# xavenordu/Audio-Compression

Measured on AMD Instinct MI355X. Metric: ranges matched/sec at tile_size=2048, top-K=64, higher is better.
Workload: dtype f32; 1 GPU; cfg2: 60 s 44100 Hz mono white noise, tile_size=2048, top_k=64, n_ranges=330750, n_domains=1321977; tile_size=2048, top_k=64, n_ranges=330750, n_domains=1321977, parallelism=single GPU, streams=2

## Files before the change

audio-compression_amd/csrc/fwav_topk.hip:

```cpp
#include <algorithm>
#include <cstring>
#include <type_traits>
#include "fwav_common.h"
#include "../../include/fwav.h"

#if !defined(FWAV_DEBUG_API) && (defined(FWAV_TOPK_ABL) || defined(FWAV_TOPK_APPOFF) || defined(FWAV_TOPK_CAP) || \
    defined(FWAV_TOPK_CB) || defined(FWAV_TOPK_CENT) || defined(FWAV_TOPK_CENTWIDE) || defined(FWAV_TOPK_CENT_HL) || \
    defined(FWAV_TOPK_CENT_MINQ) || defined(FWAV_TOPK_CG) || defined(FWAV_TOPK_CHAINS) || \
    defined(FWAV_TOPK_CPDBL) || defined(FWAV_TOPK_CPMIN) || defined(FWAV_TOPK_CSHARE) || defined(FWAV_TOPK_BANDB) || defined(FWAV_TOPK_CVACC) || \
    defined(FWAV_TOPK_CW) || defined(FWAV_TOPK_CWPE) || defined(FWAV_TOPK_DELTA) || defined(FWAV_TOPK_EXGROW) || \
    defined(FWAV_TOPK_EXWPE) || defined(FWAV_TOPK_FIRST) || defined(FWAV_TOPK_G) || defined(FWAV_TOPK_GROW) || \
    defined(FWAV_TOPK_HLDELTA) || defined(FWAV_TOPK_HLPRE) || defined(FWAV_TOPK_INTERLEAVE) || \
    defined(FWAV_TOPK_MAXP) || defined(FWAV_TOPK_PMAJOR) || defined(FWAV_TOPK_PRIO) || defined(FWAV_TOPK_QS) || \
    defined(FWAV_TOPK_RB) || defined(FWAV_TOPK_SEEDHALF) || defined(FWAV_TOPK_SMALLSORT) || defined(FWAV_TOPK_W) || \
    defined(FWAV_TOPK_WARM) || defined(FWAV_TOPK_WIDE_MIN) || defined(FWAV_TOPK_WIN) || defined(FWAV_TOPK_WPE) || \
    defined(FWAV_FLOOR_PILOTS) || defined(FWAV_FLOOR_RANK) || defined(FWAV_TOPK_YOUNG) || defined(FWAV_TOPK_TAIL))
#error "experiment switches build the debug library only (-DFWAV_DEBUG_API)"
#endif

namespace fwav {

typedef float floatx16 __attribute__((ext_vector_type(16)));

constexpr int kTopkWaves = 4;
constexpr int kTopkQ = 32 * kTopkWaves;
constexpr int kChunk = 256;
constexpr int kTopkThreads = 64 * kTopkWaves;

__device__ __forceinline__ uint64_t make_key(float s, int32_t idx) {
  return ((uint64_t)f2key(s) << 32) | (uint64_t)(~(uint32_t)idx);
}
__device__ __forceinline__ int32_t key_idx(uint64_t k) { return (int32_t)(~(uint32_t)(k & 0xffffffffu)); }
__device__ __forceinline__ float key_score(uint64_t k) { return key2f((uint32_t)(k >> 32)); }

template <int E>
__device__ __forceinline__ void wave_sort_desc(uint64_t (&v)[E]) {
  const int lane = threadIdx.x & 63;
  constexpr int N = E * 64;
#pragma unroll
  for (int size = 2; size <= N; size <<= 1) {
#pragma unroll
    for (int stride = size >> 1; stride > 0; stride >>= 1) {
      if (stride >= 64) {
        const int js = stride >> 6;
#pragma unroll
        for (int j = 0; j < E; ++j) {
          if ((j & js) == 0) {
            const int jp = j | js;
            const int e = j * 64 + lane;
            const bool desc = (e & size) == 0;
            uint64_t a = v[j], b = v[jp];
            bool sw = desc ? (a < b) : (a > b);
            v[j] = sw ? b : a;
            v[jp] = sw ? a : b;
          }
        }
      } else {
#pragma unroll
        for (int j = 0; j < E; ++j) {
          const int e = j * 64 + lane;
          uint64_t o = __shfl_xor(v[j], stride);
          const bool lower = (lane & stride) == 0;
          const bool desc = (e & size) == 0;
          uint64_t mx = v[j] > o ? v[j] : o;
          uint64_t mn = v[j] > o ? o : v[j];
          v[j] = (lower == desc) ? mx : mn;
        }
      }
    }
  }
}

template <int E>
__device__ __forceinline__ int tie_flags(const uint64_t (&v)[E], int n, int K) {
  const int lane = threadIdx.x & 63;
  bool in = false, bd = false;
#pragma unroll
  for (int j = 0; j < E; ++j) {
    uint64_t nx = __shfl_down(v[j], 1);
    const uint64_t first_next = __shfl(v[j + 1 < E ? j + 1 : j], 0);
    if (lane == 63) nx = j + 1 < E ? first_next : 0ull;
    const int e = j * 64 + lane;
    if (e + 1 < n && e + 1 <= K && key_score(nx) == key_score(v[j])) {
      if (e + 1 < K) in = true;
      else bd = true;
    }
  }
  return (__ballot(in) != 0ull ? 1 : 0) | (__ballot(bd) != 0ull ? 2 : 0);
}

template <int E>
__device__ __forceinline__ void record_tie(int32_t* ties, int32_t qid, int flags, const uint64_t (&v)[E], int n,
                                           int K, bool group) {
  if (ties == nullptr || flags == 0) return;
  const int lane = threadIdx.x & 63;
  int pos = 0;
  if (lane == 0) pos = atomicAdd(ties, 1);
  pos = __shfl(pos, 0);
  int32_t* rec = ties + 1 + (int64_t)kTieRec * pos;
  if (lane == 0) rec[0] = 2 * qid + ((flags >> 1) & 1);
  if (!(flags & 2)) return;
  int total = -1;
  if (group) {
    uint64_t kth = 0;
#pragma unroll
    for (int j = 0; j < E; ++j)
      if (j == ((K - 1) >> 6)) kth = __shfl(v[j], (K - 1) & 63);
    const float S = key_score(kth);
    total = 0;
#pragma unroll
    for (int j = 0; j < E; ++j) {
      const int e = j * 64 + lane;
      const bool in = e >= K && e < n && key_score(v[j]) == S;
      if (in && e - K < kTieRec - 2) rec[2 + e - K] = key_idx(v[j]);
      total += __popcll(__ballot(in));
    }
    if (total > kTieRec - 2) total = -1;
  }
  if (lane == 0) rec[1] = total;
}
template <int E>
__device__ __forceinline__ void record_tie(int32_t* ties, int32_t qid, int flags, const uint64_t (&v)[E], int n,
                                           int K) {
  record_tie<E>(ties, qid, flags, v, n, K, false);
}

template <int C>
__device__ __forceinline__ int compact(uint64_t* __restrict__ keys, int* __restrict__ cnt, float* __restrict__ theta,
                                       int ql, int K) {
  constexpr int E = C / 64;
  const int lane = threadIdx.x & 63;
  const int n = cnt[ql];
  uint64_t v[E];
#pragma unroll
  for (int j = 0; j < E; ++j) {
    const int e = j * 64 + lane;
    v[j] = e < n ? keys[ql * C + e] : 0ull;
  }
  wave_sort_desc<E>(v);
  const int tf = tie_flags<E>(v, n, K);
#pragma unroll
  for (int j = 0; j < E; ++j) {
    const int e = j * 64 + lane;
    if (e < K && e < n) keys[ql * C + e] = v[j];
  }
  const int kl = (K - 1) & 63, kj = (K - 1) >> 6;
  uint64_t kth = 0;
#pragma unroll
  for (int j = 0; j < E; ++j)
    if (j == kj) kth = __shfl(v[j], kl);
  if (lane == 0) {
    cnt[ql] = n < K ? n : K;
    theta[ql] = n >= K ? key_score(kth) : -INFINITY;
  }
  return tf;
// ... 818 lines not shown
      stat_add(11, __builtin_amdgcn_s_memrealtime() - t_l0);
    }
#pragma unroll
    for (int u = 0; u < kReplayBatch; ++u) {
      if (ct[u] < 0) break;
      floatx16 acc = __builtin_amdgcn_mfma_f32_32x32x16_f16(af[u], b, floatx16{}, 0, 0, 0);
      if constexpr (HL) {
#if FWAV_TOPK_HLPRE
        if (__ballot(fold16((int)0x80000000, acc) > int_threshold(thf - kStreamMargin)) == 0ull) continue;
#endif
        acc = __builtin_amdgcn_mfma_f32_32x32x16_f16(af[u], bl, acc, 0, 0, 0);
        acc = __builtin_amdgcn_mfma_f32_32x32x16_f16(afl[u], b, acc, 0, 0, 0);
      }
      thf = append_tile<C, STATS, SM, MODE>(acc, thf, qcnt, kept, ct[u], nd, gkeys, sm, qg, K, upd, stats, sp, emb,
                                          qv, kthp, share);
    }
    if (ct[kReplayBatch - 1] < 0) break;
  }
  return thf;
}

#ifndef FWAV_TOPK_SEEDHALF
#define FWAV_TOPK_SEEDHALF 64
#endif
constexpr int kSeedHalf = FWAV_TOPK_SEEDHALF;
constexpr int kSeedTiles = (2 * kSeedHalf + 62) / 32 + 1;
template <int MODE>
__device__ __forceinline__ float seed_limit(const _Float16* __restrict__ emb16, int64_t nd, half8 b, int64_t qrow,
                                            int64_t wbase, int K) {
  const int lane = threadIdx.x & 63;
  const int col = lane & 31;
  const int h = lane >> 5;
  const half8* afp[kSeedTiles];
  uint32_t wm[kSeedTiles];
#pragma unroll
  for (int t = 0; t < kSeedTiles; ++t) {
    const int64_t dt = wbase + 32 * t;
    const bool ok = dt >= 0 && dt < nd;
    const int64_t c = ok ? dt / kChunk : 0, tt = ok ? (dt % kChunk) / 32 : 0;
    afp[t] = reinterpret_cast<const half8*>(emb16 + ((c * 2 + h) * kChunk + col) * 8 + tt * 256);
    uint32_t m = 0;
#pragma unroll
    for (int r = 0; r < 16; ++r) {
      const int64_t d = dt + 4 * h + (r & 3) + 8 * (r >> 2);
      m |= (ok && d < nd && d >= qrow - kSeedHalf && d < qrow + kSeedHalf) ? (1u << r) : 0u;
    }
    wm[t] = m;
  }
  auto count_ge = [&](float thr) {
    int c = 0;
    half8 af[kSeedTiles];
#pragma unroll
    for (int t = 0; t < kSeedTiles; ++t) af[t] = *afp[t];
#pragma unroll
    for (int t = 0; t < kSeedTiles; ++t) {
      const floatx16 acc = __builtin_amdgcn_mfma_f32_32x32x16_f16(af[t], b, floatx16{}, 0, 0, 0);
#pragma unroll
      for (int r = 0; r < 16; ++r) c += ((wm[t] >> r) & 1u) && acc[r] >= thr ? 1 : 0;
    }
    return c + __shfl_xor(c, 32);
  };
  const bool ok = count_ge(0.0f) >= K;
  uint32_t T = 0x80000000u;
  for (int bit = 30; bit >= 12; --bit) {
    const uint32_t Tc = T | (1u << bit);
    const int c = count_ge(key2f(Tc));
    T = c >= K ? Tc : T;
  }
  return ok ? (MODE == kModeHL ? key2f(T) - kF16Delta - 2.0f * kHLDelta : key2f(T) - 2.0f * kF16Delta) : -INFINITY;
}

template <int NC, int QS, int MODE = 0>
__device__ __forceinline__ void stream_group(const _Float16* __restrict__ lda0, const half8 (&b)[QS],
                                             const int (&thi)[QS], int cbase, uint32_t (*fired)[kFifo],
                                             int (&nfired)[QS], int lane, int* sink = nullptr) {
  constexpr int NT = 8 * NC;
  constexpr int kChunkHalfs = 512 * 8;
  auto chunk_of = [](int i) { return i >> 3; };
  auto rd = [&](int i) {
    return *reinterpret_cast<const half8*>(lda0 + chunk_of(i) * kChunkHalfs + (i & 7) * 256);
  };
  half8 a[NT];
  floatx16 acc[NT][QS];
#pragma unroll
  for (int i = 0; i < 3 && i < NT; ++i) a[i] = rd(i);
#pragma unroll
  for (int s = 0; s < QS; ++s) acc[0][s] = __builtin_amdgcn_mfma_f32_32x32x16_f16(a[0], b[s], floatx16{}, 0, 0, 0);
  int r[QS][kChains];
#pragma unroll
  for (int s = 0; s < QS; ++s)
#pragma unroll
    for (int c = 0; c < kChains; ++c) r[s][c] = (int)0x80000000;
#pragma unroll
  for (int i = 0; i < NT; ++i) {
    if (i + 3 < NT) a[i + 3] = rd(i + 3);
#pragma unroll
    for (int s = 0; s < QS; ++s) {
      if (i + 1 < NT) acc[i + 1][s] = __builtin_amdgcn_mfma_f32_32x32x16_f16(a[i + 1], b[s], floatx16{}, 0, 0, 0);
      constexpr int cm = kChains - 1;
      if (MODE & 2)
        r[s][i & cm] = max(max(r[s][i & cm], __float_as_int(acc[i][s][0])), __float_as_int(acc[i][s][15]));
      else
        r[s][i & cm] = fold16(r[s][i & cm], acc[i][s]);
    }
    if (MODE != 0) {
      if (i == NT - 1) {
#pragma unroll
        for (int s = 0; s < QS; ++s)
#pragma unroll
          for (int c = 0; c < kChains; ++c) *sink ^= r[s][c];
      }
      continue;
    }
    if ((i & 7) == 7) {
#pragma unroll
      for (int s = 0; s < QS; ++s) {
        const int t = thi[s];
        int rm = r[s][0];
#pragma unroll
        for (int c = 1; c < kChains; ++c) rm = max(rm, r[s][c]);
        if (__ballot(rm > t) != 0ull) {
          uint32_t mk = 0u;
#pragma unroll
          for (int c = 0; c < kChains; ++c) mk |= __ballot(r[s][c] > t) != 0ull ? (1u << c) : 0u;
          if (lane == 0) fired[s][nfired[s] & (kFifo - 1)] = ((uint32_t)(cbase + chunk_of(i)) << 8) | mk;
          ++nfired[s];
        }
#pragma unroll
        for (int c = 0; c < kChains; ++c) r[s][c] = (int)0x80000000;
      }
    }
  }
}

__device__ __forceinline__ int ctz_mask(uint32_t x) { return __builtin_ctz(x); }
__device__ __forceinline__ int ctz_mask(uint64_t x) { return __builtin_ctzll(x); }
template <int N, int I = 0, class F>
__device__ __forceinline__ void static_for(F&& f) {
  if constexpr (I < N) {
    f(std::integral_constant<int, I>{});
    static_for<N, I + 1>(f);
  }
}

constexpr int kCentBatch = FWAV_TOPK_CB;
template <int QS>
__device__ __forceinline__ uint64_t cent_set_mask(int s) {
  static_assert(QS == 2 || QS == 4 || QS == 8, "centroid sets: 2, 4 or 8 query sets per wave");
  constexpr uint64_t m = QS == 2 ? 0x5555555555555555ull : (QS == 4 ? 0x1111111111111111ull : 0x0101010101010101ull);
  return m << s;
}
template <int QS, class RowOf>
__device__ __forceinline__ void centroid_setup(const _Float16* __restrict__ emb16, RowOf qrow_of, half8& bc,
                                               float& slack) {
  typedef float floatx8 __attribute__((ext_vector_type(8)));
  const int lane = threadIdx.x & 63;
  const int h = lane >> 5;
  auto frag = [&](int64_t r) {
    return *reinterpret_cast<const half8*>(emb16 + (((r >> 8) * 2 + h) * 256 + (r & 255)) * 8);
  };
  floatx8 sum = {0.f, 0.f, 0.f, 0.f, 0.f, 0.f, 0.f, 0.f};
  int nv = 0;
#pragma unroll
  for (int k = 0; k < QS; ++k) {
    const int64_t r = qrow_of(k);
    if (r >= 0) {
      const half8 m = frag(r);
      ++nv;
#pragma unroll
      for (int i = 0; i < 8; ++i) sum[i] += (float)m[i];
    }
  }
  half8 c;
#pragma unroll
  for (int i = 0; i < 8; ++i) c[i] = (_Float16)(nv > 0 ? sum[i] / (float)nv : 0.0f);
  float rho = 0.0f;
#pragma unroll
  for (int k = 0; k < QS; ++k) {
    const int64_t r = qrow_of(k);
    if (r >= 0) {
      const half8 m = frag(r);
      float d2 = 0.0f;
#pragma unroll
      for (int i = 0; i < 8; ++i) {
        const float d = (float)m[i] - (float)c[i];
        d2 += d * d;
      }
      rho = fmaxf(rho, __builtin_sqrtf(d2));
    }
  }
  rho += __shfl_xor(rho, 32);
  bc = c;
  slack = rho * (1.0f + 0x1p-9f) + 1e-5f;
}
template <int QS>
__device__ __forceinline__ int centroid_threshold(const float (&tv)[QS], float slack) {
  const int lane = threadIdx.x & 63;
  const int col = lane & 31;
  const int sj = col % QS, base = (lane & 32) + QS * (col / QS);
  float mn = INFINITY;
#pragma unroll
  for (int k = 0; k < QS; ++k) {
    float v = INFINITY;
#pragma unroll
    for (int s = 0; s < QS; ++s) {
      const float x = __shfl(tv[s], base + k);
      v = s == sj ? x : v;
    }
    mn = fminf(mn, v);
  }
  return int_threshold(mn - slack);
}
template <int NC, int QS>
__device__ __forceinline__ void cent_level1(const _Float16* __restrict__ lda0, half8 bc, int thc,
                                            uint64_t (&pend)[QS]) {
  constexpr int NT = 8 * NC;
  static_assert(NT <= 64, "tile masks are 64-bit");
  constexpr int kChunkHalfs = 512 * 8;
  auto rd = [&](int i) {
    return *reinterpret_cast<const half8*>(lda0 + (i >> 3) * kChunkHalfs + (i & 7) * 256);
  };
#pragma unroll
  for (int s = 0; s < QS; ++s) pend[s] = 0ull;
  half8 a[NT];
  floatx16 acc[NT];
#pragma unroll
  for (int i = 0; i < 3 && i < NT; ++i) a[i] = rd(i);
  acc[0] = __builtin_amdgcn_mfma_f32_32x32x16_f16(a[0], bc, floatx16{}, 0, 0, 0);
if constexpr (FWAV_TOPK_CVACC && NT <= 32) {
  uint32_t bits = 0u;
#pragma unroll
  for (int i = 0; i < NT; ++i) {
    if (i + 3 < NT) a[i + 3] = rd(i + 3);
    if (i + 1 < NT) acc[i + 1] = __builtin_amdgcn_mfma_f32_32x32x16_f16(a[i + 1], bc, floatx16{}, 0, 0, 0);
    const uint64_t m = __ballot(fold16((int)0x80000000, acc[i]) > thc);
    uint64_t co;
    asm("v_addc_co_u32_e64 %0, %1, %2, %2, %3" : "=v"(bits), "=s"(co) : "v"(bits), "s"(m));
  }
#pragma unroll
  for (int off = QS; off < 64; off <<= 1) bits |= (uint32_t)__shfl_xor((int)bits, off);
#pragma unroll
  for (int s = 0; s < QS; ++s)
    pend[s] = (uint64_t)(__builtin_bitreverse32((uint32_t)__builtin_amdgcn_readlane((int)bits, s)) >> (32 - NT));
} else {
#pragma unroll
  for (int i = 0; i < NT; ++i) {
    if (i + 3 < NT) a[i + 3] = rd(i + 3);
    if (i + 1 < NT) acc[i + 1] = __builtin_amdgcn_mfma_f32_32x32x16_f16(a[i + 1], bc, floatx16{}, 0, 0, 0);
    const uint64_t m = __ballot(fold16((int)0x80000000, acc[i]) > thc);
#pragma unroll
    for (int s = 0; s < QS; ++s)
      if (m & cent_set_mask<QS>(s)) pend[s] |= 1ull << i;
  }
}
}

template <int C, bool STATS, int MODE, int W = k16Waves, int G = kGroup, int QS = k16Sets, bool CENT = false>
__global__ __launch_bounds__(64 * W, MODE == kModeEX ? FWAV_TOPK_EXWPE : (CENT ? FWAV_TOPK_CWPE : FWAV_TOPK_WPE)) void k_sim_topk_f16(const _Float16* __restrict__ emb16,
                                                                const float* __restrict__ emb, int64_t nd,
                                                                const int32_t* __restrict__ active,
                                                                const int32_t* __restrict__ n_active_p,
                                                                int64_t q_offset, int K, int32_t* __restrict__ cand,
                                                                uint64_t* __restrict__ gkeys_all,
                                                                int32_t* __restrict__ ovf_list,
                                                                int32_t* __restrict__ n_ovf,
                                                                uint32_t* __restrict__ share_lim,
                                                                const uint32_t* __restrict__ seeds_in,
                                                                float seed_shift, int plan_rt,
                                                                int plan_p, int dbg, unsigned long long* gstats,
                                                                SgemvSplit sp, int32_t* __restrict__ ties,
                                                                FloorCtl fl) {
  constexpr bool EX = MODE == kModeEX;
  constexpr bool HL = MODE == kModeHL;
  constexpr int NG = W * QS;
  constexpr bool ABL = STATS || FWAV_TOPK_ABL != 0;
  constexpr int NB = 2;
  struct Lds {
    u32x4 slots[NB * G][512];
    Topk16SmemT<NG, STATS, !CENT, W> sm;
  };
  __shared__ __attribute__((aligned(16))) Lds lds_all;
  u32x4(*slots)[512] = lds_all.slots;
  Topk16SmemT<NG, STATS, !CENT, W>& sm = lds_all.sm;

  const int n_active = *n_active_p;
  constexpr int QB = 32 * NG;
  const uint32_t fkey = (!EX && fl.key != nullptr) ? __builtin_amdgcn_readfirstlane(*fl.key) : 0u;
  const bool alt = fl.key != nullptr && fkey == 0u;
  const TopkPlan plan = make_plan(n_active, alt ? fl.alt_rt : plan_rt, alt ? fl.alt_p : plan_p, QB);
  int64_t block;
  int piece, npieces, qhalf;
  plan_item(plan, blockIdx.x, block, piece, npieces, qhalf);
  if (block >= plan.nb) return;
  const int Wact = qhalf < 0 ? W : W / 2;
  if ((int)(threadIdx.x >> 6) >= Wact) return;
  const int qslot0 = qhalf > 0 ? (W / 2) * QS * 32 : 0;
  uint64_t* gkeys = gkeys_all + (size_t)blockIdx.x * 32 * NG * C;
  const unsigned long long t_kernel = STATS ? __builtin_amdgcn_s_memrealtime() : 0;

  const int tid = threadIdx.x;
  const int lane = tid & 63;
  const int wave = __builtin_amdgcn_readfirstlane(tid >> 6);
  unsigned long long* stats = nullptr;
  if (STATS) {
    if (lane < kStats) sm.wstat[wave][lane] = 0;
    stats = sm.wstat[wave];
  }
  const int col = lane & 31;
  const int h = lane >> 5;
  if (!STATS) dbg = FWAV_TOPK_ABL;
  half8 b[QS], bl[QS];
  float thf[QS];
  int upd[QS];
  float qv[QS][EX ? 16 : 1];
  const int64_t n16 = (int64_t)cdiv(nd, kChunk) * kChunk * 16;
  const _Float16* emb16lo = emb16 + n16;
  uint64_t kth[QS];
  float inseed[QS];
  int32_t qpos[QS];
  uint32_t* share = (npieces > 1 && !EX) ? share_lim : nullptr;
#pragma unroll
  for (int s = 0; s < QS; ++s) {
    const int ql = (wave * QS + s) * 32 + col;
    const int64_t qi = slot_query(block, qslot0 + ql, plan.nb, QB);
    const int32_t q = qi < n_active ? active[qi] : -1;
    const int64_t qrow = (int64_t)(q < 0 ? 0 : q) + q_offset;
    b[s] = *reinterpret_cast<const half8*>(emb16 + (((qrow >> 8) * 2 + h) * 256 + (qrow & 255)) * 8);
    bl[s] = *reinterpret_cast<const half8*>(emb16lo + (((qrow >> 8) * 2 + h) * 256 + (qrow & 255)) * 8);
    upd[s] = (q >= 0 && !(dbg & 1)) ? 1 : 0;
    thf[s] = upd[s] ? -INFINITY : INFINITY;
    qpos[s] = (int32_t)(qi < n_active ? qi : 0);
    if (h == 0) {
      sm.ovf[ql] = 0;
      sm.tie[ql] = 0;
      sm.qrow[ql] = qrow;
      sm.qpos[ql] = qpos[s];
    }
    kth[s] = 0ull;
    inseed[s] = seeds_in != nullptr && q >= 0 ? key2f(seeds_in[qi]) - seed_shift : -INFINITY;
    if constexpr (EX) {
      const float* qp = emb + qrow * 16;
#pragma unroll
      for (int i = 0; i < 16; ++i) qv[s][i] = qp[i];
    }
  }

  if (!(ABL && (dbg & 8192))) {
#pragma unroll
    for (int s = 0; s < QS; ++s) {
      const int64_t wbase =
          (int64_t)((__builtin_amdgcn_readfirstlane((int)sm.qrow[(wave * QS + s) * 32]) - kSeedHalf) >> 5) << 5;
      const float seed = seed_limit<MODE>(emb16, nd, b[s], sm.qrow[(wave * QS + s) * 32 + col], wbase, K);
      if (upd[s]) thf[s] = seed;
      if (STATS && (dbg & 32768) && gstats != nullptr && h == 0 && upd[s])
        gstats[16 + slot_query(block, qslot0 + (wave * QS + s) * 32 + col, plan.nb, QB)] = __float_as_uint(seed);
    }
  }
  if (seeds_in != nullptr) {
#pragma unroll
    for (int s = 0; s < QS; ++s)
      if (upd[s]) thf[s] = fmaxf(thf[s], inseed[s]);
  }
  if (fkey != 0u) {
#pragma unroll
    for (int s = 0; s < QS; ++s)
      if (upd[s]) thf[s] = fmaxf(thf[s], key2f(fkey));
  }
  int lid[QS];
#pragma unroll
  for (int s = 0; s < QS; ++s) lid[s] = wave * QS + s;
  half8 bc{};
  float cslack = 0.0f;
  auto setup_centroids = [&]() {
    const int sj = col % QS, mcol0 = QS * (col / QS);
    int ls = lid[0];
#pragma unroll
    for (int s = 1; s < QS; ++s) ls = sj == s ? lid[s] : ls;
    centroid_setup<QS>(emb16, [&](int k) -> int64_t {
      const int64_t qi = slot_query(block, qslot0 + ls * 32 + mcol0 + k, plan.nb, QB);
      return qi < n_active ? (int64_t)active[qi] + q_offset : (int64_t)-1;
    }, bc, cslack);
  };
  if constexpr (CENT) setup_centroids();
  const int nchunks = (int)cdiv(nd, kChunk);
  if ((FWAV_TOPK_PRIO & 1) && wave >= W / 2) __builtin_amdgcn_s_setprio(1);
  int c0, c1;
  piece_chunks(plan, block, piece, npieces, nchunks, c0, c1);
  const int ngroups = (c1 - c0 + G - 1) / G;
  const u32x4* src = reinterpret_cast<const u32x4*>(emb16);
  auto issue_group = [&](int gg) {
#pragma unroll
    for (int j = 0; j < G; ++j) {
      int c_ = c0 + gg * G + j;
      c_ = c_ < c1 ? c_ : c1 - 1;
      if (ABL && (dbg & 4)) c_ = 0;
      if (ABL && (dbg & 128) && (j & 1)) continue;
      for (int k = wave; k < 8; k += Wact) {
        const unsigned lds_dst = __builtin_amdgcn_readfirstlane((unsigned)(size_t)(
            (__attribute__((address_space(3))) void*)(&slots[(gg % NB) * G + j][k * 64])));
        const u32x4* gsrc = src + (int64_t)c_ * 512 + k * 64 + lane;
        unsigned keep;
        asm volatile("s_mov_b32 %0, m0\n\ts_mov_b32 m0, %2\n\ts_nop 0\n\tglobal_load_lds_dwordx4 %1, off\n\ts_mov_b32 m0, %0"
                     : "=&s"(keep) : "v"(gsrc), "s"(lds_dst) : "memory");
      }
    }
  };
  __builtin_amdgcn_s_waitcnt(0x0F70);
  if (ngroups > 0) issue_group(0);

  int sink = 0;
  int nfired[QS];
  ReplayCursor cur[QS];
  int qcnt[QS];
  int kept[QS];
#pragma unroll
  for (int s = 0; s < QS; ++s) {
    nfired[s] = qcnt[s] = kept[s] = 0;
    cur[s] = ReplayCursor{0, 0, 0u};
  }
  uint32_t shv[QS];
  for (int g = 0; g < ngroups; ++g) {
    u32x4(*half)[512] = slots + (g % NB) * G;
    const int cg = c0 + g * G;
    const int c_end = cg + G < c1 ? cg + G : c1;
    const bool window_end =
        (c_end - c0 <= kWarmChunks) || ((g + 1) % (kWindowGroups * 4 / G) == 0) || (g + 1 == ngroups);
    if (CENT && FWAV_TOPK_CSHARE && share != nullptr) {
#pragma unroll
      for (int s = 0; s < QS; ++s)
        shv[s] = __hip_atomic_load(share + qpos[s], __ATOMIC_RELAXED, __HIP_MEMORY_SCOPE_AGENT);
    }
    const unsigned long long t_b0 = STATS ? __builtin_amdgcn_s_memrealtime() : 0;
    if (!(ABL && (dbg & 256))) {
      asm volatile("s_waitcnt vmcnt(0) lgkmcnt(0)" ::: "memory");
      if (STATS) stat_add(12, __builtin_amdgcn_s_memrealtime() - t_b0);
      if (FWAV_TOPK_PRIO & 4) __builtin_amdgcn_s_setprio(0);
      if (!(ABL && (dbg & 16384))) __builtin_amdgcn_s_barrier();
      asm volatile("" ::: "memory");
    }
    const unsigned long long t_b1 = STATS ? __builtin_amdgcn_s_memrealtime() : 0;
    if (STATS) stat_add(7, t_b1 - t_b0);
    if (CENT && FWAV_TOPK_CSHARE && share != nullptr) {
#pragma unroll
      for (int s = 0; s < QS; ++s)
        if (upd[s] && shv[s] != 0u) thf[s] = fmaxf(thf[s], key2f(shv[s]));
    }
    if (g + 1 < ngroups) issue_group(g + 1);
    if (ABL && (dbg & 2)) continue;
    int thi[QS];
#pragma unroll
    for (int s = 0; s < QS; ++s) thi[s] = int_threshold(HL ? thf[s] - kStreamMargin : thf[s]);
    const _Float16* lda0 = reinterpret_cast<const _Float16*>(half[0]) + ((h * kChunk) + col) * 8;
    if constexpr (CENT) {
      float tv[QS];
#pragma unroll
      for (int s = 0; s < QS; ++s) tv[s] = HL ? thf[s] - kStreamMargin : thf[s];
      const int thc = centroid_threshold<QS>(tv, cslack);
      uint64_t pend[QS];
      const unsigned long long t_l1 = STATS ? __builtin_amdgcn_s_memrealtime() : 0;
      if (c_end - cg == G) {
        cent_level1<G, QS>(lda0, bc, thc, pend);
      } else {
#pragma unroll
        for (int s = 0; s < QS; ++s) pend[s] = 0ull;
        for (int c = cg; c < c_end; ++c) {
          uint64_t pc[QS];
          cent_level1<1, QS>(lda0 + (c - cg) * 512 * 8, bc, thc, pc);
#pragma unroll
          for (int s = 0; s < QS; ++s) pend[s] |= pc[s] << (8 * (c - cg));
        }
      }
      if (STATS) {
        stat_add(13, __builtin_amdgcn_s_memrealtime() - t_l1);
        unsigned long long np = 0;
#pragma unroll
        for (int s = 0; s < QS; ++s) np += __popcll(pend[s]);
        stat_add(14, np);
      }
      if (FWAV_TOPK_PRIO & 4) __builtin_amdgcn_s_setprio(1);
      static_for<QS>([&](auto sc) {
        constexpr int s = decltype(sc)::value;
        using TMask = uint64_t;
        TMask pm = (TMask)pend[s];
        TMask pass = 0;
        while (pm != 0) {
          int t[kCentBatch];
          bool on[kCentBatch];
#pragma unroll
          for (int u = 0; u < kCentBatch; ++u) {
            on[u] = pm != 0;
            t[u] = on[u] ? ctz_mask(pm) : t[0];
            if (on[u]) pm &= pm - 1;
          }
          half8 af[kCentBatch];
          floatx16 acc[kCentBatch];
#pragma unroll
          for (int u = 0; u < kCentBatch; ++u)
            af[u] = *reinterpret_cast<const half8*>(lda0 + (t[u] >> 3) * (512 * 8) + (t[u] & 7) * 256);
#pragma unroll
          for (int u = 0; u < kCentBatch; ++u)
            acc[u] = __builtin_amdgcn_mfma_f32_32x32x16_f16(af[u], b[s], floatx16{}, 0, 0, 0);
#pragma unroll
          for (int u = 0; u < kCentBatch; ++u) {
            if (!on[u]) break;
            if constexpr (HL) {
              if (__ballot(fold16((int)0x80000000, acc[u]) > thi[s]) != 0ull) pass |= (TMask)1 << t[u];
            } else {
              const int64_t dt = (int64_t)(cg + (t[u] >> 3)) * kChunk + (t[u] & 7) * 32;
              thf[s] = append_tile<C, STATS, Topk16SmemT<NG, STATS, !CENT, W>, MODE>(acc[u], thf[s], qcnt[s], kept[s],
                                                                                 dt, nd, gkeys, sm, lid[s], K,
                                                                                 upd[s], stats, sp, emb, qv[s],
                                                                                 &kth[s], share);
            }
          }
        }
        if constexpr (HL) {
          while (pass != 0) {
            int t[kReplayBatch];
            bool on[kReplayBatch];
#pragma unroll
            for (int u = 0; u < kReplayBatch; ++u) {
              on[u] = pass != 0;
              t[u] = on[u] ? ctz_mask(pass) : t[0];
              if (on[u]) pass &= pass - 1;
            }
            half8 afl[kReplayBatch];
#pragma unroll
            for (int u = 0; u < kReplayBatch; ++u)
              afl[u] = tile_fragment(emb16lo, (int64_t)(cg + (t[u] >> 3)) * kChunk + (t[u] & 7) * 32, h, col);
#pragma unroll
            for (int u = 0; u < kReplayBatch; ++u) {
              if (!on[u]) break;
              const half8 af = *reinterpret_cast<const half8*>(lda0 + (t[u] >> 3) * (512 * 8) + (t[u] & 7) * 256);
              floatx16 a2 = __builtin_amdgcn_mfma_f32_32x32x16_f16(af, b[s], floatx16{}, 0, 0, 0);
              a2 = __builtin_amdgcn_mfma_f32_32x32x16_f16(af, bl[s], a2, 0, 0, 0);
              a2 = __builtin_amdgcn_mfma_f32_32x32x16_f16(afl[u], b[s], a2, 0, 0, 0);
              const int64_t dt = (int64_t)(cg + (t[u] >> 3)) * kChunk + (t[u] & 7) * 32;
              thf[s] = append_tile<C, STATS, Topk16SmemT<NG, STATS, !CENT, W>, MODE>(a2, thf[s], qcnt[s], kept[s], dt,
                                                                                 nd, gkeys, sm, lid[s], K,
                                                                                 upd[s], stats, sp, emb, qv[s],
                                                                                 &kth[s], share);
            }
          }
        }
      });
    } else if (ABL && (dbg & (512 | 1024)) && c_end - cg == G) {
      if (dbg & 1024)
        stream_group<G, QS, 2>(lda0, b, thi, cg, sm.fired + wave * QS, nfired, lane, &sink);
      else
        stream_group<G, QS, 1>(lda0, b, thi, cg, sm.fired + wave * QS, nfired, lane, &sink);
    } else if (c_end - cg == G) {
      stream_group<G, QS>(lda0, b, thi, cg, sm.fired + wave * QS, nfired, lane);
    } else {
      for (int c = cg; c < c_end; ++c)
        stream_group<1, QS>(lda0 + (c - cg) * 512 * 8, b, thi, c, sm.fired + wave * QS, nfired, lane);
    }
    const unsigned long long t_c = STATS ? __builtin_amdgcn_s_memrealtime() : 0;
    if (STATS) stat_add(9, t_c - t_b1);
    if (window_end) {
      if (share != nullptr && !(CENT && FWAV_TOPK_CSHARE)) {
#pragma unroll
        for (int s = 0; s < QS; ++s) {
          const uint32_t v = __hip_atomic_load(share + qpos[s], __ATOMIC_RELAXED, __HIP_MEMORY_SCOPE_AGENT);
          if (upd[s] && v != 0u) thf[s] = fmaxf(thf[s], key2f(v));
        }
      }
      if (!CENT && (FWAV_TOPK_PRIO & 8)) __builtin_amdgcn_s_setprio(1);
      static_for<QS>([&](auto sc) {
        constexpr int s = decltype(sc)::value;
        if constexpr (!CENT) {
          if (nfired[s] > cur[s].head || cur[s].rem != 0u)
            thf[s] = replay_window<C, STATS, Topk16SmemT<NG, STATS, !CENT, W>, MODE>(emb16, emb16lo, b[s], bl[s], thf[s],
                                             qcnt[s], kept[s], cur[s], nfired[s], nd, gkeys, sm, lid[s], K, upd[s],
                                             stats, sp, emb, qv[s], &kth[s], share);
        }
      });
      if (!CENT && (FWAV_TOPK_PRIO & 8)) __builtin_amdgcn_s_setprio(0);
      if (STATS) stat_add(4, __builtin_amdgcn_s_memrealtime() - t_c);
      __builtin_amdgcn_s_waitcnt(0x0F70);
    }
  }
  const unsigned long long t_final = STATS ? __builtin_amdgcn_s_memrealtime() : 0;
#pragma unroll
  for (int s = 0; s < QS; ++s) {
    if (h == 0)
      sm.cnt[lid[s] * 32 + col] = qcnt[s];
    else
      sm.cnt1[lid[s] * 32 + col] = qcnt[s];
  }

  auto slot_of = [&](int l) {
    int ls = lid[0];
#pragma unroll
    for (int s = 1; s < QS; ++s) ls = (l >> 5) == s ? lid[s] : ls;
    return ls * 32 + (l & 31);
  };
  if (npieces > 1) {
    asm volatile("s_waitcnt vmcnt(0)" ::: "memory");
    for (int l0 = 0; l0 < 32 * QS; l0 += kBandBatch) {
      uint64_t v[kBandBatch][C / 64];
      int nb_[kBandBatch];
      uint32_t sh[kBandBatch];
#pragma unroll
      for (int b = 0; b < kBandBatch; ++b) {
        const int qs = slot_of(l0 + b);
        const int64_t qq = slot_query(block, qslot0 + qs, plan.nb, QB);
        const bool ok = l0 + b < 32 * QS && qq < n_active;
        nb_[b] = ok ? piece_band_load<C>(gkeys + (size_t)qs * C, sm, qs, v[b]) : -1;
        sh[b] = ok ? __hip_atomic_load(share_lim + qq, __ATOMIC_RELAXED, __HIP_MEMORY_SCOPE_AGENT) : 0u;
      }
#pragma unroll
      for (int b = 0; b < kBandBatch; ++b) {
        if (nb_[b] < 0) continue;
        const int qs = slot_of(l0 + b);
        const int64_t qq = slot_query(block, qslot0 + qs, plan.nb, QB);
        if (lane == 0) FWAV_TRACE(sm.qrow[qs], 3u, (uint32_t)sm.cnt[qs], (uint32_t)sm.ovf[qs], (uint32_t)sm.cnt1[qs]);
        piece_band<C, HL>(gkeys + (size_t)qs * C, sm, qs, K, share_lim + qq, v[b], nb_[b], sh[b]);
      }
    }
  }
  for (int l = 0; l < (npieces > 1 ? 0 : 32 * QS); ++l) {
    const int qs = slot_of(l);
    const int64_t qq = slot_query(block, qslot0 + qs, plan.nb, QB);
    if (qq >= n_active) continue;
    const int32_t qid = active[qq];
    uint64_t* kq = gkeys + (size_t)qs * C;
    if (lane == 0) FWAV_TRACE(sm.qrow[qs], 3u, (uint32_t)sm.cnt[qs], (uint32_t)sm.ovf[qs], (uint32_t)sm.cnt1[qs]);
    compact16<C>(kq, sm, qs, K, emb, cand + (int64_t)qid * K, sp, ties, qid, fkey, fl);
    if (lane == 0 && sm.ovf[qs]) {
      const int pos = atomicAdd(n_ovf, 1);
      ovf_list[pos] = qid;
      reinterpret_cast<uint32_t*>(n_ovf + 1)[pos] = (uint32_t)sm.ovf[qs];
    }
  }
  if (ABL && sink == 0x7fffffff) cand[0] = sink;
  if (STATS) {
    stat_add(8, __builtin_amdgcn_s_memrealtime() - t_final);
    stat_add(6, __builtin_amdgcn_s_memrealtime() - t_kernel);
    __syncthreads();
    if (gstats != nullptr && threadIdx.x == 0) {
      unsigned long long mx = 0;
      for (int w = 0; w < Wact; ++w) mx = max(mx, sm.wstat[w][6] - sm.wstat[w][7]);
      atomicAdd(gstats + 15, mx);
    }
    if (gstats != nullptr && lane < kStats && lane != 15) atomicAdd(gstats + lane, sm.wstat[wave][lane]);
    if (gstats != nullptr && (dbg & 4096) && lane == 0) {
      atomicMin(gstats + 16 + 2 * blockIdx.x, t_kernel);
      atomicMax(gstats + 17 + 2 * blockIdx.x, __builtin_amdgcn_s_memrealtime());
    }
  }
}

template <int E>
__device__ __forceinline__ void merge_band(const uint64_t* __restrict__ sw, int mb, int K, const float* __restrict__ emb,
                                           int64_t qrow, const SgemvSplit& sp, int32_t* __restrict__ ties, int32_t qid,
                                           int32_t* __restrict__ out, uint32_t fkey, const FloorCtl& fl) {
  const int lane = threadIdx.x & 63;
  uint64_t v[E];
#pragma unroll
  for (int j = 0; j < E; ++j) {
    const int e = j * 64 + lane;
    v[j] = e < mb ? sw[e] : 0ull;
  }
  const float4* qp = reinterpret_cast<const float4*>(emb + qrow * 16);
  float qv[16];
#pragma unroll
  for (int i = 0; i < 4; ++i) {
    const float4 x = qp[i];
    qv[4 * i] = x.x; qv[4 * i + 1] = x.y; qv[4 * i + 2] = x.z; qv[4 * i + 3] = x.w;
  }
#pragma unroll
  for (int j0 = 0; j0 < E; j0 += 2) {
    float4 row[2][4];
    int32_t dd[2];
#pragma unroll
    for (int jj = 0; jj < 2; ++jj) {
      const int j = j0 + jj < E ? j0 + jj : E - 1;
      dd[jj] = (j0 + jj < E && v[j] != 0ull) ? key_idx(v[j]) : 0;
      const float4* rp = reinterpret_cast<const float4*>(emb + (int64_t)dd[jj] * 16);
#pragma unroll
      for (int i = 0; i < 4; ++i) row[jj][i] = rp[i];
    }
#pragma unroll
    for (int jj = 0; jj < 2; ++jj) {
      const int j = j0 + jj;
      if (j < E && v[j] != 0ull) {
        const float acc = sgemv16([&](int k) { return f4c(row[jj][k >> 2], k & 3); }, [&](int k) { return qv[k]; },
                                  sgemv_kind((uint32_t)dd[jj], sp));
        v[j] = make_key(acc, dd[jj]);
      }
    }
  }
  wave_sort_desc<E>(v);
  if (fkey != 0u) {
// ... 1086 lines not shown
```

Measured before the change: 25.33 million ranges/s.

## Tighten centroid pruning bound with direction decomposition and cache the threshold

Replaces the plain radius slack of the centroid lower bound with a tighter bound that splits each query's offset from the centroid into a part along the centroid and a part perpendicular to it. The aim is a higher centroid threshold, so fewer tiles pass level-1 filtering and need per-query MFMA and top-k appends. It also caches the centroid threshold and recomputes it only when some query's running threshold changed, which costs extra ballots after each append. The new bound adds per-setup arithmetic and relies on careful floating-point safety margins to stay exact.

```diff
diff --git a/audio-compression_amd/csrc/fwav_centroid_bound.h b/audio-compression_amd/csrc/fwav_centroid_bound.h
--- /dev/null
+++ b/audio-compression_amd/csrc/fwav_centroid_bound.h
@@ -0,0 +1,87 @@
+#ifndef FWAV_CENTROID_BOUND_H
+#define FWAV_CENTROID_BOUND_H
+
+#include <cmath>
+
+#if defined(__HIPCC__) || defined(__CUDACC__)
+#define FWAV_HD __host__ __device__
+#else
+#define FWAV_HD
+#endif
+
+namespace fwav {
+
+constexpr float kCentD = 1.0f + 0x1p-9f;
+constexpr float kCentEta = 1e-5f;
+
+struct CentHead {
+  float n2, rho, beta, perp2;
+};
+struct CentBound {
+  float slack, gd, k0, k2;
+};
+
+FWAV_HD inline float cent_rcp(float x) {
+#if defined(__HIP_DEVICE_COMPILE__)
+  return __builtin_amdgcn_rcpf(x);
+#else
+  return 1.0f / x;
+#endif
+}
+FWAV_HD inline float cent_sqrt(float x) {
+#if defined(__HIP_DEVICE_COMPILE__)
+  return __builtin_amdgcn_sqrtf(x);
+#else
+  return sqrtf(x);
+#endif
+}
+
+FWAV_HD inline void cent_head_begin(CentHead& t, const float (&c)[8]) {
+  float n2 = 0.0f;
+  for (int i = 0; i < 8; ++i) n2 += c[i] * c[i];
+  t = CentHead{n2, 0.0f, 0.0f, 0.0f};
+}
+FWAV_HD inline void cent_head_member(CentHead& t, const float (&c)[8], const float (&q)[8]) {
+  float e2 = 0.0f, ec = 0.0f;
+  for (int i = 0; i < 8; ++i) {
+    const float e = q[i] - c[i];
+    e2 += e * e;
+    ec += e * c[i];
+  }
+  const float en = sqrtf(e2);
+  t.rho = fmaxf(t.rho, en);
+  float b2 = 0.0f;
+  if (t.n2 > 0.0f) {
+    b2 = fminf(ec * ec / t.n2, e2);
+    t.beta = fmaxf(t.beta, sqrtf(b2) + 0x1p-20f * en);
+  }
+  t.perp2 = fmaxf(t.perp2, (e2 - b2) + 0x1p-18f * e2);
+}
+FWAV_HD inline CentBound cent_bound(const CentHead& h0, const CentHead& h1) {
+  CentBound b;
+  b.slack = (h0.rho + h1.rho) * kCentD + kCentEta;
+  const float N2 = (h0.n2 + h1.n2) * (1.0f - 0x1p-20f);
+  const float s2 = (h0.perp2 + h1.perp2) * (1.0f + 0x1p-20f);
+  if (N2 > 0.0f) {
+    b.gd = (h0.beta + h1.beta) * kCentD + kCentEta;
+    b.k0 = 2.0f * s2 * (kCentD * kCentD);
+    b.k2 = s2 / N2;
+  } else {
+    b.gd = INFINITY;
+    b.k0 = b.k2 = 0.0f;
+  }
+  return b;
+}
+FWAV_HD inline float cent_threshold(const CentBound& b, float tmin, bool tight = true) {
+  const float old = tmin - b.slack;
+  const float t = tmin - b.gd;
+  if (!tight || !(t > 0.0f) || !(t < INFINITY)) return old;
+  const float A = 1.0f + b.k2;
+  const float rad = fmaxf(b.k0 * A * (1.0f + 0x1p-12f) - b.k2 * (t * t), 0.0f);
+  const float s = (t - cent_sqrt(rad)) * cent_rcp(A);
+  return s > 0.0f ? fmaxf(old, s) : old;
+}
+
+}
+
+#endif
diff --git a/audio-compression_amd/csrc/fwav_topk.hip b/audio-compression_amd/csrc/fwav_topk.hip
--- a/audio-compression_amd/csrc/fwav_topk.hip
+++ b/audio-compression_amd/csrc/fwav_topk.hip
@@ -1,6 +1,7 @@
 #include <algorithm>
 #include <cstring>
 #include <type_traits>
+#include "fwav_centroid_bound.h"
 #include "fwav_common.h"
 #include "../../include/fwav.h"
 
@@ -1125,7 +1126,7 @@
 }
 template <int QS, class RowOf>
 __device__ __forceinline__ void centroid_setup(const _Float16* __restrict__ emb16, RowOf qrow_of, half8& bc,
-                                               float& slack) {
+                                               CentBound& cb) {
   typedef float floatx8 __attribute__((ext_vector_type(8)));
   const int lane = threadIdx.x & 63;
   const int h = lane >> 5;
@@ -1145,29 +1146,32 @@
     }
   }
   half8 c;
-#pragma unroll
-  for (int i = 0; i < 8; ++i) c[i] = (_Float16)(nv > 0 ? sum[i] / (float)nv : 0.0f);
-  float rho = 0.0f;
+  float cf[8];
+#pragma unroll
+  for (int i = 0; i < 8; ++i) {
+    c[i] = (_Float16)(nv > 0 ? sum[i] / (float)nv : 0.0f);
+    cf[i] = (float)c[i];
+  }
+  CentHead own;
+  cent_head_begin(own, cf);
 #pragma unroll
   for (int k = 0; k < QS; ++k) {
     const int64_t r = qrow_of(k);
     if (r >= 0) {
       const half8 m = frag(r);
-      float d2 = 0.0f;
-#pragma unroll
-      for (int i = 0; i < 8; ++i) {
-        const float d = (float)m[i] - (float)c[i];
-        d2 += d * d;
-      }
-      rho = fmaxf(rho, __builtin_sqrtf(d2));
-    }
-  }
-  rho += __shfl_xor(rho, 32);
+      float mf[8];
+#pragma unroll
+      for (int i = 0; i < 8; ++i) mf[i] = (float)m[i];
+      cent_head_member(own, cf, mf);
+    }
+  }
+  const CentHead oth{__shfl_xor(own.n2, 32), __shfl_xor(own.rho, 32), __shfl_xor(own.beta, 32),
+                     __shfl_xor(own.perp2, 32)};
   bc = c;
-  slack = rho * (1.0f + 0x1p-9f) + 1e-5f;
+  cb = cent_bound(own, oth);
 }
 template <int QS>
-__device__ __forceinline__ int centroid_threshold(const float (&tv)[QS], float slack) {
+__device__ __forceinline__ int centroid_threshold(const float (&tv)[QS], const CentBound& cb, bool tight) {
   const int lane = threadIdx.x & 63;
   const int col = lane & 31;
   const int sj = col % QS, base = (lane & 32) + QS * (col / QS);
@@ -1182,7 +1186,7 @@
     }
     mn = fminf(mn, v);
   }
-  return int_threshold(mn - slack);
+  return int_threshold(cent_threshold(cb, mn, tight));
 }
 template <int NC, int QS>
 __device__ __forceinline__ void cent_level1(const _Float16* __restrict__ lda0, half8 bc, int thc,
@@ -1343,7 +1347,7 @@
 #pragma unroll
   for (int s = 0; s < QS; ++s) lid[s] = wave * QS + s;
   half8 bc{};
-  float cslack = 0.0f;
+  CentBound cb{};
   auto setup_centroids = [&]() {
     const int sj = col % QS, mcol0 = QS * (col / QS);
     int ls = lid[0];
@@ -1352,7 +1356,7 @@
     centroid_setup<QS>(emb16, [&](int k) -> int64_t {
       const int64_t qi = slot_query(block, qslot0 + ls * 32 + mcol0 + k, plan.nb, QB);
       return qi < n_active ? (int64_t)active[qi] + q_offset : (int64_t)-1;
-    }, bc, cslack);
+    }, bc, cb);
   };
   if constexpr (CENT) setup_centroids();
   const int nchunks = (int)cdiv(nd, kChunk);
@@ -1392,6 +1396,8 @@
     cur[s] = ReplayCursor{0, 0, 0u};
   }
   uint32_t shv[QS];
+  int thc = 0;
+  bool thc_stale = true;
   for (int g = 0; g < ngroups; ++g) {
     u32x4(*half)[512] = slots + (g % NB) * G;
     const int cg = c0 + g * G;
@@ -1415,8 +1421,11 @@
     if (STATS) stat_add(7, t_b1 - t_b0);
     if (CENT && FWAV_TOPK_CSHARE && share != nullptr) {
 #pragma unroll
-      for (int s = 0; s < QS; ++s)
+      for (int s = 0; s < QS; ++s) {
+        const float t0 = thf[s];
         if (upd[s] && shv[s] != 0u) thf[s] = fmaxf(thf[s], key2f(shv[s]));
+        thc_stale |= __ballot(thf[s] != t0) != 0ull;
+      }
     }
     if (g + 1 < ngroups) issue_group(g + 1);
     if (ABL && (dbg & 2)) continue;
@@ -1425,10 +1434,13 @@
     for (int s = 0; s < QS; ++s) thi[s] = int_threshold(HL ? thf[s] - kStreamMargin : thf[s]);
     const _Float16* lda0 = reinterpret_cast<const _Float16*>(half[0]) + ((h * kChunk) + col) * 8;
     if constexpr (CENT) {
-      float tv[QS];
-#pragma unroll
-      for (int s = 0; s < QS; ++s) tv[s] = HL ? thf[s] - kStreamMargin : thf[s];
-      const int thc = centroid_threshold<QS>(tv, cslack);
+      if (thc_stale) {
+        float tv[QS];
+#pragma unroll
+        for (int s = 0; s < QS; ++s) tv[s] = HL ? thf[s] - kStreamMargin : thf[s];
+        thc = centroid_threshold<QS>(tv, cb, !(ABL && (dbg & 2048)));
+        thc_stale = false;
+      }
       uint64_t pend[QS];
       const unsigned long long t_l1 = STATS ? __builtin_amdgcn_s_memrealtime() : 0;
       if (c_end - cg == G) {
@@ -1480,10 +1492,12 @@
               if (__ballot(fold16((int)0x80000000, acc[u]) > thi[s]) != 0ull) pass |= (TMask)1 << t[u];
             } else {
               const int64_t dt = (int64_t)(cg + (t[u] >> 3)) * kChunk + (t[u] & 7) * 32;
+              const float t0 = thf[s];
               thf[s] = append_tile<C, STATS, Topk16SmemT<NG, STATS, !CENT, W>, MODE>(acc[u], thf[s], qcnt[s], kept[s],
                                                                                  dt, nd, gkeys, sm, lid[s], K,
                                                                                  upd[s], stats, sp, emb, qv[s],
                                                                                  &kth[s], share);
+              thc_stale |= __ballot(thf[s] != t0) != 0ull;
             }
           }
         }
@@ -1509,10 +1523,12 @@
               a2 = __builtin_amdgcn_mfma_f32_32x32x16_f16(af, bl[s], a2, 0, 0, 0);
               a2 = __builtin_amdgcn_mfma_f32_32x32x16_f16(afl[u], b[s], a2, 0, 0, 0);
               const int64_t dt = (int64_t)(cg + (t[u] >> 3)) * kChunk + (t[u] & 7) * 32;
+              const float t0 = thf[s];
               thf[s] = append_tile<C, STATS, Topk16SmemT<NG, STATS, !CENT, W>, MODE>(a2, thf[s], qcnt[s], kept[s], dt,
                                                                                  nd, gkeys, sm, lid[s], K,
                                                                                  upd[s], stats, sp, emb, qv[s],
                                                                                  &kth[s], share);
+              thc_stale |= __ballot(thf[s] != t0) != 0ull;
             }
           }
         }
```

Measured after the change: 26.87 million ranges/s (median of 6 runs). 6.1% higher.
